# CX9898/BSMR-SDDMM

Hardware: AMD Instinct MI355X
Metric: SDDMM GFLOP/s (higher is better)
Workload: dtype f16

## Files before the change

### bsmr-sddmm_amd/csrc/gemm_kernels.hpp

```cpp
#pragma once

#include <hip/hip_runtime.h>
#include <stdint.h>

#include "gemm_format.hpp"
#include "sddmm_kernels.hpp"

namespace bsmr {

constexpr uint32_t kGemmBK = 64;
constexpr uint32_t kGemmRowBytes = kGemmBK * 2u;
__host__ __device__ constexpr uint32_t gemmSwz16(uint32_t row) { return (row >> 1) & 7u; }
__host__ __device__ constexpr uint32_t gemmSwz32(uint32_t row) { return ((row >> 1) & 1u) | (((row >> 3) & 1u) * 6u); }
constexpr uint32_t gemmStageBytes(int PM, int NB) { return (uint32_t)(PM + NB) * 16u * kGemmRowBytes; }
constexpr uint32_t kGemmSlabBytes = kGemmPassTiles * 1024u;
constexpr uint32_t gemmRingBytes(int PM, int NB) {
    return 2u * gemmStageBytes(PM, NB) > kGemmWaves * kGemmSlabBytes ? 2u * gemmStageBytes(PM, NB) : kGemmWaves * kGemmSlabBytes;
}
constexpr size_t gemmLdsBytes(int PM, int NB) { return gemmRingBytes(PM, NB) + (size_t)PM * 16u * 4u; }

#if defined(BSMR_GEMM_LAB)
#define GEMM_LAB_ARG , uint32_t labSkip, unsigned long long* labStamps
#define GEMM_LAB_SKIP(bit) (labSkip & (1u << (bit)))
#define GEMM_LAB_STAMPS unsigned long long labStamp[8] = {0, 0, 0, 0, 0, 0, 0, 0}
#define GEMM_LAB_STAMP(i) labStamp[i] = __builtin_amdgcn_s_memrealtime()
#define GEMM_LAB_STAMPS_OUT                                                                              \
    if (labStamps && lane == 0)                                                                          \
        for (uint32_t i = 0; i < 8u; ++i) labStamps[((size_t)blockIdx.x * kGemmWaves + wave) * 8u + i] = labStamp[i]
#else
#define GEMM_LAB_ARG
#define GEMM_LAB_SKIP(bit) false
#define GEMM_LAB_STAMPS
#define GEMM_LAB_STAMP(i)
#define GEMM_LAB_STAMPS_OUT
#endif

__device__ __forceinline__ void gemmKeep(const u32x4& x) {
#if defined(__HIP_DEVICE_COMPILE__)
    asm volatile("" ::"v"(x));
#else
    (void)x;
#endif
}

constexpr uint32_t kGemmDumpHigh = 64764u;
__device__ __forceinline__ void gemmDumpTile(const f32x4& a, uint32_t tileAddr, bool high) {
#if defined(__HIP_DEVICE_COMPILE__)
#pragma clang diagnostic push
#pragma clang diagnostic ignored "-Winline-asm"
    if (!high)
        asm volatile("s_mov_b32 m0, %4\n\ts_nop 0\n\tds_write_addtid_b32 %0\n\tds_write_addtid_b32 %1 offset:256\n\t"
                     "ds_write_addtid_b32 %2 offset:512\n\tds_write_addtid_b32 %3 offset:768"
                     ::"v"(a[0]), "v"(a[1]), "v"(a[2]), "v"(a[3]), "s"(tileAddr) : "memory", "m0");
    else
        asm volatile("s_mov_b32 m0, %4\n\ts_nop 0\n\tds_write_addtid_b32 %0 offset:64764\n\tds_write_addtid_b32 %1 offset:65020\n\t"
                     "ds_write_addtid_b32 %2 offset:65276\n\tds_write_addtid_b32 %3 offset:65532"
                     ::"v"(a[0]), "v"(a[1]), "v"(a[2]), "v"(a[3]), "s"(tileAddr - kGemmDumpHigh) : "memory", "m0");
#pragma clang diagnostic pop
#else
    (void)a; (void)tileAddr; (void)high;
#endif
}
__device__ __forceinline__ uint32_t gemmLdsAddress(const void* p) {
    return (uint32_t)(uintptr_t)(__attribute__((address_space(3))) const void*)p;
}

template <uint32_t DMAS>
__device__ __forceinline__ void gemmStagePart(const uint8_t* src, uint32_t srcBytes, uint8_t* dst, uint32_t wave, const uint32_t* voff, uint32_t kOff) {
    const auto rsrc = __builtin_amdgcn_make_buffer_rsrc(const_cast<uint8_t*>(src), 0, srcBytes, 0x00020000);
#pragma unroll
    for (uint32_t j = 0; j < DMAS; ++j)
        __builtin_amdgcn_raw_ptr_buffer_load_lds(rsrc, (__attribute__((address_space(3))) void*)(dst + (wave * DMAS + j) * 1024u), 16, voff[j], kOff, 0, 0);
}
__device__ __forceinline__ void gemmStoreEntry(float* P, bool live, uint32_t index, float val) {
    const auto rsrc = __builtin_amdgcn_make_buffer_rsrc(P, 0, 0xFFFFFFFC, 0x00020000);
    __builtin_amdgcn_raw_buffer_store_b32(__builtin_bit_cast(uint32_t, val), rsrc, live ? index << 2 : 0xFFFFFFFFu, 0, 0);
}
template <uint32_t C>
__device__ __forceinline__ void gemmLoadWords(const uint32_t* __restrict__ words, uint32_t e0, uint32_t lane, uint32_t (&w)[C], bool skip) {
    const uint32_t* __restrict__ base = words + e0;
#pragma unroll
    for (uint32_t u = 0; u < C; ++u) w[u] = skip ? kGemmNoEntry : base[u * kWave + lane];
}
template <uint32_t C, uint32_t HALF>
__device__ __forceinline__ void gemmMaskTrip(const float* slab, const uint32_t* rowTable, float* P, uint32_t e, uint32_t last, uint32_t lane,
                                             const uint32_t (&w)[C], bool skipStores) {
#pragma unroll
    for (uint32_t u = 0; u < C; ++u) {
        const bool live = e + u * kWave + lane < last && w[u] != kGemmNoEntry;
        const float val = slab[w[u] & 4095u];
        const uint32_t dst = rowTable[(w[u] >> 12) & (HALF - 1u)] + (w[u] >> 19);
        if (!skipStores) gemmStoreEntry(P, live, dst, val);
    }
}
template <uint32_t C, uint32_t HALF, uint32_t Q, bool DEEP>
__device__ __forceinline__ void gemmMaskPass(const uint32_t* __restrict__ words, const float* slab, const uint32_t* rowTable, float* P,
                                             const uint32_t (&myList)[Q + 1u], uint32_t q, uint32_t lane, uint32_t (&wAhead)[2][C],
                                             bool skipLoads, bool skipStores) {
    const uint32_t first = myList[q], last = myList[q + 1u];
    uint32_t w[C];
#pragma unroll
    for (uint32_t u = 0; u < C; ++u) w[u] = wAhead[q & 1u][u];
    if (DEEP) {
        if (q + 2u < Q) gemmLoadWords<C>(words, myList[q + 2u], lane, wAhead[q & 1u], skipLoads);
    } else if (q + 1u < Q) {
        gemmLoadWords<C>(words, last, lane, wAhead[(q + 1u) & 1u], skipLoads);
    }
    constexpr uint32_t T = C * kWave;
    const bool more = first + T < last;
    uint32_t over[C];
    if (more) gemmLoadWords<C>(words, first + T, lane, over, skipLoads);
    gemmMaskTrip<C, HALF>(slab, rowTable, P, first, last, lane, w, skipStores);
    if (more) {
        for (uint32_t e = first + T; e < last; e += T) {
            uint32_t ahead[C];
            gemmLoadWords<C>(words, e + T, lane, ahead, skipLoads);
            gemmMaskTrip<C, HALF>(slab, rowTable, P, e, last, lane, over, skipStores);
#pragma unroll
            for (uint32_t u = 0; u < C; ++u) over[u] = ahead[u];
        }
    }
}
template <uint32_t ADMAS, uint32_t BDMAS>
__device__ __forceinline__ void gemmStage(const uint8_t* A, uint32_t aBytes, const uint8_t* B, uint32_t bBytes, uint8_t* stage, uint32_t bAt,
                                          uint32_t wave, const uint32_t* voffA, const uint32_t* voffB, uint32_t kOff) {
    gemmStagePart<BDMAS>(B, bBytes, stage + bAt, wave, voffB, kOff);
    gemmStagePart<ADMAS>(A, aBytes, stage, wave, voffA, kOff);
}
__device__ __forceinline__ uint32_t gemmRowOfLane(const uint32_t* __restrict__ rows8, uint32_t sub) {
    uint32_t id = rows8[0];
#pragma unroll
    for (uint32_t k = 1; k < 8; ++k) id = sub == k ? rows8[k] : id;
    return id;
}

template <int KT, int PM, int NB, int MODE, bool SRC32 = false>
__global__ void __launch_bounds__(kGemmWaves * kWave, 2)
denseGemm(const void* __restrict__ Aop, const void* __restrict__ Bop, uint32_t aBytes, uint32_t bBytes,
          const uint32_t* __restrict__ panelRows, const uint32_t* __restrict__ colOf, const GemmItem* __restrict__ items,
          const uint32_t* __restrict__ rowStart,
          const uint32_t* __restrict__ lists, const uint32_t* __restrict__ words, float* __restrict__ P, uint32_t N,
          uint32_t gridG, uint32_t gridS, uint32_t fullGrid, Batch batch GEMM_LAB_ARG) {
    constexpr uint32_t ESZ = SRC32 ? 4u : 2u, K = (kGemmRowBytes / ESZ) * KT, TM = PM * 16u, TN = NB * 16u;
    constexpr uint32_t KSUB = SRC32 ? 1u : 2u;
    constexpr uint32_t m = PM / kGemmWavesM, n = NB / kGemmWavesN, Q = (m * n + kGemmPassTiles - 1u) / kGemmPassTiles, L = kGemmWaves * Q;
    constexpr uint32_t ADMAS = PM / 4u, BDMAS = NB / 4u;
    static_assert(PM % 4 == 0 && NB % 4 == 0, "a stage is filled in whole 1-KiB pieces per wave");
    constexpr uint32_t stageBytes = gemmStageBytes(PM, NB), bAt = TM * kGemmRowBytes;
    constexpr uint32_t rowTableAt = gemmRingBytes(PM, NB);
    constexpr uint32_t kGemmWordChunk = m * n > 32u ? 4u : 8u;
    constexpr bool kPlainDump = m * n > 32u;

    extern __shared__ __attribute__((aligned(16))) uint8_t lds[];
    const uint32_t itemId = xcdContiguous(blockIdx.x, gridDim.x);
    uint32_t group, firstBlock, listBase;
    if (fullGrid) {
        gemmItemPlace(itemId, gridG, gridS, group, firstBlock);
        firstBlock *= (uint32_t)NB;
        listBase = itemId * (L + 1u);
    } else {
        const GemmItem item = items[itemId];
        group = item.group;
        firstBlock = item.firstBlock;
        listBase = item.listBase;
    }
    const uint32_t wave = __builtin_amdgcn_readfirstlane(threadIdx.x >> 6), lane = threadIdx.x & 63u;
    const uint32_t wm = wave / kGemmWavesN, wn = wave % kGemmWavesN;
    const uint32_t r = lane & 15u, g = lane >> 4;
    GEMM_LAB_STAMPS;
    GEMM_LAB_STAMP(0);

    const uint8_t* Ab = static_cast<const uint8_t*>(Aop) + (size_t)blockIdx.y * batch.strideA * ESZ;
    const uint8_t* Bb = static_cast<const uint8_t*>(Bop) + (size_t)blockIdx.y * batch.strideB * ESZ;
    P += (size_t)blockIdx.y * batch.strideP;

    uint32_t voffA[ADMAS], voffB[BDMAS];
#pragma unroll
    for (uint32_t j = 0; j < BDMAS; ++j) {
        const uint32_t col = 8u * (wave * BDMAS + j) + (lane >> 3);
        const uint32_t id = gemmRowOfLane(colOf + (size_t)firstBlock * 16u + 8u * (wave * BDMAS + j), lane >> 3);
        voffB[j] = id * (K * ESZ) + (((lane & 7u) ^ (SRC32 ? gemmSwz32(col) : gemmSwz16(col))) << 4);
    }
    if (!GEMM_LAB_SKIP(2)) gemmStagePart<BDMAS>(Bb, bBytes, lds + bAt, wave, voffB, 0u);
#pragma unroll
    for (uint32_t j = 0; j < ADMAS; ++j) {
        const uint32_t row = 8u * (wave * ADMAS + j) + (lane >> 3);
        const uint32_t id = gemmRowOfLane(panelRows + (size_t)group * TM + 8u * (wave * ADMAS + j), lane >> 3);
        voffA[j] = id * (K * ESZ) + (((lane & 7u) ^ (SRC32 ? gemmSwz32(row) : gemmSwz16(row))) << 4);
    }
    if (!GEMM_LAB_SKIP(2)) gemmStagePart<ADMAS>(Ab, aBytes, lds, wave, voffA, 0u);
    GEMM_LAB_STAMP(1);
    if (threadIdx.x < TM) reinterpret_cast<uint32_t*>(lds + rowTableAt)[threadIdx.x] = rowStart[(size_t)itemId * TM + threadIdx.x];
    uint32_t myList[Q + 1];
#pragma unroll
    for (uint32_t q = 0; q <= Q; ++q) myList[q] = lists[listBase + wave * Q + q];

    const uint32_t fragOff = r * kGemmRowBytes + ((SRC32 ? (2u * g) ^ gemmSwz32(r) : g ^ gemmSwz16(r)) << 4);
    const uint32_t aRead = wm * (TM / 2u) * kGemmRowBytes + fragOff;
    const uint32_t bRead = bAt + wn * (TN / 4u) * kGemmRowBytes + fragOff;

    f32x4 acc[m][n];
#pragma unroll
    for (uint32_t i = 0; i < m; ++i)
#pragma unroll
        for (uint32_t j = 0; j < n; ++j) acc[i][j] = f32x4{0.f, 0.f, 0.f, 0.f};

    auto loadWords = [&](uint32_t e0, uint32_t (&w)[kGemmWordChunk]) { gemmLoadWords<kGemmWordChunk>(words, e0, lane, w, GEMM_LAB_SKIP(4)); };
    constexpr bool kDeepWords = Q >= 2u && m * n <= 32u;
    uint32_t wAhead[2][kGemmWordChunk];
    constexpr bool kEarlyWords = KT <= 4 && !kPlainDump;
    auto firstWords = [&]() {
        loadWords(myList[0], wAhead[0]);
        if (kDeepWords) loadWords(myList[1], wAhead[1]);
    };
#if !defined(BSMR_GEMM_LATE_WORDS)
    if (kEarlyWords) firstWords();
#endif

    asm volatile("s_waitcnt vmcnt(0)" ::: "memory");
    GEMM_LAB_STAMP(2);
    __builtin_amdgcn_s_barrier();
    GEMM_LAB_STAMP(3);
#if defined(BSMR_GEMM_LATE_WORDS)
    if (kEarlyWords) firstWords();
#endif

#pragma unroll
    for (uint32_t t = 0; t < (uint32_t)KT; ++t) {
        if (t + 1u < (uint32_t)KT && !GEMM_LAB_SKIP(2))
            gemmStage<ADMAS, BDMAS>(Ab, aBytes, Bb, bBytes, lds + ((t + 1u) & 1u) * stageBytes, bAt, wave, voffA, voffB, (t + 1u) * kGemmRowBytes);
        if (!kEarlyWords && t + 1u == (uint32_t)KT) firstWords();
        const uint8_t* base = lds + (t & 1u) * stageBytes;
#pragma unroll
        for (uint32_t s = 0; s < KSUB; ++s) {
            auto fragment = [&](uint32_t at, uint32_t tile, uint32_t tag) -> u32x4 {
                if (GEMM_LAB_SKIP(1)) return u32x4{lane, t, tile, s + tag};
                const uint8_t* src = base + ((at + tile * 16u * kGemmRowBytes) ^ (s << 6));
                if constexpr (SRC32) {
                    const f32x4 lo = *reinterpret_cast<const f32x4*>(src);
                    const f32x4 hi = *reinterpret_cast<const f32x4*>(reinterpret_cast<const uint8_t*>(reinterpret_cast<uintptr_t>(src) ^ 16u));
                    return packLowp<MODE>(lo, hi);
                } else {
                    return *reinterpret_cast<const u32x4*>(src);
                }
            };
            u32x4 bf[n];
#pragma unroll
            for (uint32_t j = 0; j < n; ++j) bf[j] = fragment(bRead, j, 0u);
#pragma unroll
            for (uint32_t i = 0; i < m; ++i) {
                const u32x4 af = fragment(aRead, i, 2u);
                if (!GEMM_LAB_SKIP(0)) {
#pragma unroll
                    for (uint32_t j = 0; j < n; ++j) acc[i][j] = mfma16<MODE>(af, bf[j], acc[i][j]);
                } else {
                    gemmKeep(af);
#pragma unroll
                    for (uint32_t j = 0; j < n; ++j) gemmKeep(bf[j]);
                }
            }
        }
        asm volatile("s_waitcnt vmcnt(0) lgkmcnt(0)" ::: "memory");
        __builtin_amdgcn_s_barrier();
    }

    GEMM_LAB_STAMP(4);
    float* slab = reinterpret_cast<float*>(lds) + wave * (kGemmPassTiles * 256u);
    const uint32_t slabAddr = __builtin_amdgcn_readfirstlane(gemmLdsAddress(slab));
    const uint32_t* rowTable = reinterpret_cast<const uint32_t*>(lds + rowTableAt) + wm * (TM / 2u);
#pragma unroll
    for (uint32_t q = 0; q < Q; ++q) {
        if (!GEMM_LAB_SKIP(3)) {
            if (kPlainDump) {
#pragma unroll
                for (uint32_t tp = 0; tp < kGemmPassTiles; ++tp) {
                    const uint32_t tIdx = q * kGemmPassTiles + tp;
                    if (tIdx < m * n) {
#pragma unroll
                        for (uint32_t j = 0; j < 4u; ++j) slab[tp * 256u + j * 64u + lane] = acc[tIdx / n][tIdx % n][j];
                    }
                }
            } else if (slabAddr < 0x10000u) {
#pragma unroll
                for (uint32_t tp = 0; tp < kGemmPassTiles; ++tp) {
                    const uint32_t tIdx = q * kGemmPassTiles + tp;
                    if (tIdx < m * n) gemmDumpTile(acc[tIdx / n][tIdx % n], slabAddr + tp * 1024u, false);
                }
            } else {
#pragma unroll
                for (uint32_t tp = 0; tp < kGemmPassTiles; ++tp) {
                    const uint32_t tIdx = q * kGemmPassTiles + tp;
                    if (tIdx < m * n) gemmDumpTile(acc[tIdx / n][tIdx % n], slabAddr + tp * 1024u, true);
                }
            }
        }
        if (kPlainDump) __builtin_amdgcn_sched_barrier(0);
        gemmMaskPass<kGemmWordChunk, TM / 2u, Q, kDeepWords>(words, slab, rowTable, P, myList, q, lane, wAhead, GEMM_LAB_SKIP(4), GEMM_LAB_SKIP(5));
        GEMM_LAB_STAMP(5u + q);
    }
    GEMM_LAB_STAMPS_OUT;
}

constexpr uint32_t kGemmHalfRowBytes = 64u;
__host__ __device__ constexpr uint32_t gemmSwzH(uint32_t row) { return (4u - ((row >> 2) & 3u)) & 3u; }
constexpr uint32_t gemmCvtRingBytes(int PM, int NB) {
    const uint32_t used = (uint32_t)(PM + NB) * 16u * (kGemmRowBytes + 2u * kGemmHalfRowBytes);
    return used > kGemmWaves * kGemmSlabBytes ? used : kGemmWaves * kGemmSlabBytes;
}
constexpr size_t gemmCvtLdsBytes(int PM, int NB) { return gemmCvtRingBytes(PM, NB) + (size_t)PM * 16u * 4u; }

template <int KT, int PM, int NB, int MODE>
__global__ void __launch_bounds__(kGemmWaves * kWave, 2)
denseGemmCvt(const float* __restrict__ Aop, const float* __restrict__ Bop, uint32_t aBytes, uint32_t bBytes,
             const uint32_t* __restrict__ panelRows, const uint32_t* __restrict__ colOf, const GemmItem* __restrict__ items,
             const uint32_t* __restrict__ rowStart,
             const uint32_t* __restrict__ lists, const uint32_t* __restrict__ words, float* __restrict__ P, uint32_t N,
             uint32_t gridG, uint32_t gridS, uint32_t fullGrid, Batch batch GEMM_LAB_ARG) {
    constexpr uint32_t K = 32u * KT, TM = PM * 16u, TN = NB * 16u, ROWS = TM + TN;
    constexpr uint32_t m = PM / kGemmWavesM, n = NB / kGemmWavesN, Q = (m * n + kGemmPassTiles - 1u) / kGemmPassTiles, L = kGemmWaves * Q;
    constexpr uint32_t ADMAS = PM / 4u, BDMAS = NB / 4u, DMAS = ADMAS + BDMAS;
    constexpr uint32_t fBytes = ROWS * kGemmRowBytes, hBytes = ROWS * kGemmHalfRowBytes, bAtF = TM * kGemmRowBytes, bAtH = TM * kGemmHalfRowBytes;
    constexpr uint32_t hAt = fBytes, rowTableAt = gemmCvtRingBytes(PM, NB);
    constexpr uint32_t kGemmWordChunk = m * n > 32u ? 4u : 8u;

    extern __shared__ __attribute__((aligned(16))) uint8_t lds[];
    const uint32_t itemId = xcdContiguous(blockIdx.x, gridDim.x);
    uint32_t group, firstBlock, listBase;
    if (fullGrid) {
        gemmItemPlace(itemId, gridG, gridS, group, firstBlock);
        firstBlock *= (uint32_t)NB;
        listBase = itemId * (L + 1u);
    } else {
        const GemmItem item = items[itemId];
        group = item.group;
        firstBlock = item.firstBlock;
        listBase = item.listBase;
    }
    const uint32_t wave = __builtin_amdgcn_readfirstlane(threadIdx.x >> 6), lane = threadIdx.x & 63u;
    const uint32_t wm = wave / kGemmWavesN, wn = wave % kGemmWavesN;
    const uint32_t r = lane & 15u, g = lane >> 4;
    GEMM_LAB_STAMPS;
    GEMM_LAB_STAMP(0);
    const uint8_t* Ab = reinterpret_cast<const uint8_t*>(Aop) + (size_t)blockIdx.y * batch.strideA * 4u;
    const uint8_t* Bb = reinterpret_cast<const uint8_t*>(Bop) + (size_t)blockIdx.y * batch.strideB * 4u;
    P += (size_t)blockIdx.y * batch.strideP;

    uint32_t voffA[ADMAS], voffB[BDMAS];
    const uint32_t piece = lane & 7u;
#pragma unroll
    for (uint32_t j = 0; j < BDMAS; ++j)
        voffB[j] = gemmRowOfLane(colOf + (size_t)firstBlock * 16u + 8u * (wave * BDMAS + j), lane >> 3) * (K * 4u) + (piece << 4);
    if (!GEMM_LAB_SKIP(2)) gemmStagePart<BDMAS>(Bb, bBytes, lds + bAtF, wave, voffB, 0u);
#pragma unroll
    for (uint32_t j = 0; j < ADMAS; ++j)
        voffA[j] = gemmRowOfLane(panelRows + (size_t)group * TM + 8u * (wave * ADMAS + j), lane >> 3) * (K * 4u) + (piece << 4);
    if (!GEMM_LAB_SKIP(2)) gemmStagePart<ADMAS>(Ab, aBytes, lds, wave, voffA, 0u);
    GEMM_LAB_STAMP(1);
    if (threadIdx.x < TM) reinterpret_cast<uint32_t*>(lds + rowTableAt)[threadIdx.x] = rowStart[(size_t)itemId * TM + threadIdx.x];
    uint32_t myList[Q + 1];
#pragma unroll
    for (uint32_t q = 0; q <= Q; ++q) myList[q] = lists[listBase + wave * Q + q];

#if defined(BSMR_GEMM_ROUND_SERIAL)
    constexpr uint32_t kRoundBatch = 1u;
#else
    constexpr uint32_t kRoundBatch = 5u;
#endif
    const uint32_t fOfA = wave * ADMAS * 1024u + lane * 16u, fOfB = bAtF + wave * BDMAS * 1024u + lane * 16u;
    auto hOf = [&](uint32_t part, uint32_t firstChunk, uint32_t odd) {
        const uint32_t quarter = (2u * (firstChunk + odd) + (lane >> 5)) & 3u;
        return hAt + part + firstChunk * 512u + (lane >> 3) * kGemmHalfRowBytes + (((piece >> 1) ^ ((4u - quarter) & 3u)) << 4) + ((piece & 1u) << 3);
    };
    const uint32_t hOfA[2] = {hOf(0u, wave * ADMAS, 0u), hOf(0u, wave * ADMAS, 1u)};
    const uint32_t hOfB[2] = {hOf(bAtH, wave * BDMAS, 0u), hOf(bAtH, wave * BDMAS, 1u)};
    auto roundChunks = [&](uint32_t to) {
        if (GEMM_LAB_SKIP(1)) return;
#pragma unroll
        for (uint32_t j0 = 0; j0 < DMAS; j0 += kRoundBatch) {
            f32x4 v[kRoundBatch];
#pragma unroll
            for (uint32_t b = 0; b < kRoundBatch; ++b) {
                const uint32_t j = j0 + b;
                if (j >= DMAS) continue;
                v[b] = j < ADMAS ? *reinterpret_cast<const f32x4*>(lds + fOfA + j * 1024u)
                                 : *reinterpret_cast<const f32x4*>(lds + fOfB + (j - ADMAS) * 1024u);
            }
#pragma unroll
            for (uint32_t b = 0; b < kRoundBatch; ++b) {
                const uint32_t j = j0 + b;
                if (j >= DMAS) continue;
                const uint32_t jj = j < ADMAS ? j : j - ADMAS;
                uint8_t* dst = lds + (j < ADMAS ? hOfA[jj & 1u] : hOfB[jj & 1u]) + jj * 512u + to * hBytes;
                typedef uint32_t u32x2 __attribute__((ext_vector_type(2)));
                u32x2 h;
                if constexpr (MODE == 0) {
                    typedef _Float16 f16x4 __attribute__((ext_vector_type(4)));
                    f16x4 o;
                    o[0] = (_Float16)v[b][0]; o[1] = (_Float16)v[b][1]; o[2] = (_Float16)v[b][2]; o[3] = (_Float16)v[b][3];
                    h = __builtin_bit_cast(u32x2, o);
                } else {
                    typedef __bf16 bf16x4 __attribute__((ext_vector_type(4)));
                    bf16x4 o;
                    o[0] = (__bf16)v[b][0]; o[1] = (__bf16)v[b][1]; o[2] = (__bf16)v[b][2]; o[3] = (__bf16)v[b][3];
                    h = __builtin_bit_cast(u32x2, o);
                }
                *reinterpret_cast<u32x2*>(dst) = h;
            }
        }
    };

    const uint32_t fragOff = r * kGemmHalfRowBytes + ((g ^ gemmSwzH(r)) << 4);
    const uint32_t aRead = wm * (TM / 2u) * kGemmHalfRowBytes + fragOff;
    const uint32_t bRead = bAtH + wn * (TN / 4u) * kGemmHalfRowBytes + fragOff;

    f32x4 acc[m][n];
#pragma unroll
    for (uint32_t i = 0; i < m; ++i)
#pragma unroll
        for (uint32_t j = 0; j < n; ++j) acc[i][j] = f32x4{0.f, 0.f, 0.f, 0.f};
    auto loadWords = [&](uint32_t e0, uint32_t (&w)[kGemmWordChunk]) { gemmLoadWords<kGemmWordChunk>(words, e0, lane, w, GEMM_LAB_SKIP(4)); };
    constexpr bool kDeepWords = Q >= 2u && m * n <= 32u;
    uint32_t wAhead[2][kGemmWordChunk];
    constexpr bool kEarlyWords = KT <= 4;
    auto firstWords = [&]() {
        loadWords(myList[0], wAhead[0]);
        if (kDeepWords) loadWords(myList[1], wAhead[1]);
    };
#if !defined(BSMR_GEMM_LATE_WORDS)
    if (kEarlyWords) firstWords();
#endif

    asm volatile("s_waitcnt vmcnt(0)" ::: "memory");
    GEMM_LAB_STAMP(2);
    roundChunks(0u);
    asm volatile("s_waitcnt lgkmcnt(0)" ::: "memory");
    if (KT > 1 && !GEMM_LAB_SKIP(2)) gemmStage<ADMAS, BDMAS>(Ab, aBytes, Bb, bBytes, lds, bAtF, wave, voffA, voffB, kGemmRowBytes);
    __builtin_amdgcn_s_barrier();
    GEMM_LAB_STAMP(3);
#if defined(BSMR_GEMM_LATE_WORDS)
    if (kEarlyWords) firstWords();
#endif

#pragma unroll
    for (uint32_t t = 0; t < (uint32_t)KT; ++t) {
        if (!kEarlyWords && t + 1u == (uint32_t)KT) firstWords();
        const uint8_t* base = lds + hAt + (t & 1u) * hBytes;
        u32x4 bf[n];
#pragma unroll
        for (uint32_t j = 0; j < n; ++j)
            bf[j] = GEMM_LAB_SKIP(6) ? u32x4{lane, t, j, 0u} : *reinterpret_cast<const u32x4*>(base + bRead + j * 16u * kGemmHalfRowBytes);
#pragma unroll
        for (uint32_t i = 0; i < m; ++i) {
            const u32x4 af = GEMM_LAB_SKIP(6) ? u32x4{lane, t, i, 2u} : *reinterpret_cast<const u32x4*>(base + aRead + i * 16u * kGemmHalfRowBytes);
            if (!GEMM_LAB_SKIP(0)) {
#pragma unroll
                for (uint32_t j = 0; j < n; ++j) acc[i][j] = mfma16<MODE>(af, bf[j], acc[i][j]);
            } else {
                gemmKeep(af);
#pragma unroll
                for (uint32_t j = 0; j < n; ++j) gemmKeep(bf[j]);
            }
        }
        if (t + 1u < (uint32_t)KT) {
            asm volatile("s_waitcnt vmcnt(0)" ::: "memory");
            roundChunks((t + 1u) & 1u);
            asm volatile("s_waitcnt lgkmcnt(0)" ::: "memory");
            if (t + 2u < (uint32_t)KT && !GEMM_LAB_SKIP(2))
                gemmStage<ADMAS, BDMAS>(Ab, aBytes, Bb, bBytes, lds, bAtF, wave, voffA, voffB, (t + 2u) * kGemmRowBytes);
        } else {
            asm volatile("s_waitcnt lgkmcnt(0)" ::: "memory");
        }
        __builtin_amdgcn_s_barrier();
    }

    GEMM_LAB_STAMP(4);
    float* slab = reinterpret_cast<float*>(lds) + wave * (kGemmPassTiles * 256u);
    const uint32_t slabAddr = __builtin_amdgcn_readfirstlane(gemmLdsAddress(slab));
    const uint32_t* rowTable = reinterpret_cast<const uint32_t*>(lds + rowTableAt) + wm * (TM / 2u);
#pragma unroll
    for (uint32_t q = 0; q < Q; ++q) {
        if (!GEMM_LAB_SKIP(3)) {
            if (slabAddr < 0x10000u) {
#pragma unroll
                for (uint32_t tp = 0; tp < kGemmPassTiles; ++tp) {
                    const uint32_t tIdx = q * kGemmPassTiles + tp;
                    if (tIdx < m * n) gemmDumpTile(acc[tIdx / n][tIdx % n], slabAddr + tp * 1024u, false);
                }
            } else {
#pragma unroll
                for (uint32_t tp = 0; tp < kGemmPassTiles; ++tp) {
                    const uint32_t tIdx = q * kGemmPassTiles + tp;
                    if (tIdx < m * n) gemmDumpTile(acc[tIdx / n][tIdx % n], slabAddr + tp * 1024u, true);
                }
            }
        }
        gemmMaskPass<kGemmWordChunk, TM / 2u, Q, kDeepWords>(words, slab, rowTable, P, myList, q, lane, wAhead, GEMM_LAB_SKIP(4), GEMM_LAB_SKIP(5));
        GEMM_LAB_STAMP(5u + q);
    }
    GEMM_LAB_STAMPS_OUT;
}

}
```

Baseline: 15620.

## Load A fp32 slices straight into registers and deepen B staging pipeline

The fp32-input GEMM kernel no longer stages A through LDS. A slices are loaded with buffer loads directly into registers and converted to half when they land, while B keeps an fp32 double buffer in LDS and is now prefetched two slices ahead. Waits use partial vmcnt counts instead of draining everything, and the rowStart table write is deferred. This targets the full vmcnt(0) stalls and the extra LDS round trip for A, at the cost of more VGPRs, a different LDS footprint, and new lab timing spans.

```diff
diff --git a/bsmr-sddmm_amd/csrc/gemm_kernels.hpp b/bsmr-sddmm_amd/csrc/gemm_kernels.hpp
--- a/bsmr-sddmm_amd/csrc/gemm_kernels.hpp
+++ b/bsmr-sddmm_amd/csrc/gemm_kernels.hpp
@@ -20,18 +20,23 @@
 constexpr size_t gemmLdsBytes(int PM, int NB) { return gemmRingBytes(PM, NB) + (size_t)PM * 16u * 4u; }
 
 #if defined(BSMR_GEMM_LAB)
+constexpr uint32_t kGemmLabStamps = 10;
 #define GEMM_LAB_ARG , uint32_t labSkip, unsigned long long* labStamps
 #define GEMM_LAB_SKIP(bit) (labSkip & (1u << (bit)))
-#define GEMM_LAB_STAMPS unsigned long long labStamp[8] = {0, 0, 0, 0, 0, 0, 0, 0}
+#define GEMM_LAB_STAMPS unsigned long long labStamp[kGemmLabStamps] = {0, 0, 0, 0, 0, 0, 0, 0, 0, 0}, labSpan = 0
 #define GEMM_LAB_STAMP(i) labStamp[i] = __builtin_amdgcn_s_memrealtime()
+#define GEMM_LAB_SPAN_BEGIN labSpan = __builtin_amdgcn_s_memrealtime()
+#define GEMM_LAB_SPAN_END(i) labStamp[i] += __builtin_amdgcn_s_memrealtime() - labSpan
 #define GEMM_LAB_STAMPS_OUT                                                                              \
     if (labStamps && lane == 0)                                                                          \
-        for (uint32_t i = 0; i < 8u; ++i) labStamps[((size_t)blockIdx.x * kGemmWaves + wave) * 8u + i] = labStamp[i]
+        for (uint32_t i = 0; i < kGemmLabStamps; ++i) labStamps[((size_t)blockIdx.x * kGemmWaves + wave) * kGemmLabStamps + i] = labStamp[i]
 #else
 #define GEMM_LAB_ARG
 #define GEMM_LAB_SKIP(bit) false
 #define GEMM_LAB_STAMPS
 #define GEMM_LAB_STAMP(i)
+#define GEMM_LAB_SPAN_BEGIN
+#define GEMM_LAB_SPAN_END(i)
 #define GEMM_LAB_STAMPS_OUT
 #endif
 
@@ -304,10 +309,45 @@
 constexpr uint32_t kGemmHalfRowBytes = 64u;
 __host__ __device__ constexpr uint32_t gemmSwzH(uint32_t row) { return (4u - ((row >> 2) & 3u)) & 3u; }
 constexpr uint32_t gemmCvtRingBytes(int PM, int NB) {
-    const uint32_t used = (uint32_t)(PM + NB) * 16u * (kGemmRowBytes + 2u * kGemmHalfRowBytes);
+    const uint32_t used = 2u * (uint32_t)NB * 16u * kGemmRowBytes + 2u * (uint32_t)(PM + NB) * 16u * kGemmHalfRowBytes;
     return used > kGemmWaves * kGemmSlabBytes ? used : kGemmWaves * kGemmSlabBytes;
 }
 constexpr size_t gemmCvtLdsBytes(int PM, int NB) { return gemmCvtRingBytes(PM, NB) + (size_t)PM * 16u * 4u; }
+static_assert(gemmCvtLdsBytes(16, 20) <= 160u * 1024u && gemmCvtLdsBytes(16, 16) <= 160u * 1024u && gemmCvtLdsBytes(8, 20) <= 160u * 1024u &&
+              gemmCvtLdsBytes(8, 16) <= 160u * 1024u, "the fp32 kernel's LDS fits a CU's 160 KiB");
+
+template <uint32_t CHUNKS>
+__device__ __forceinline__ void gemmLoadChunks(const uint8_t* src, uint32_t srcBytes, const uint32_t* voff, uint32_t kOff, f32x4 (&v)[CHUNKS]) {
+    const auto rsrc = __builtin_amdgcn_make_buffer_rsrc(const_cast<uint8_t*>(src), 0, srcBytes, 0x00020000);
+#pragma unroll
+    for (uint32_t j = 0; j < CHUNKS; ++j) v[j] = __builtin_bit_cast(f32x4, __builtin_amdgcn_raw_buffer_load_b128(rsrc, voff[j], kOff, 0));
+}
+template <uint32_t N, uint32_t CHUNKS>
+__device__ __forceinline__ void gemmWaitRequests(f32x4 (&landed)[CHUNKS]) {
+    static_assert(N < 64u, "vmcnt holds six bits");
+    asm volatile("s_waitcnt vmcnt(%0)" ::"n"(N) : "memory");
+#if defined(__HIP_DEVICE_COMPILE__)
+#pragma unroll
+    for (uint32_t j = 0; j < CHUNKS; ++j) asm volatile("" : "+v"(landed[j]));
+#endif
+}
+template <int MODE>
+__device__ __forceinline__ void gemmRoundPiece(const f32x4& v, uint8_t* dst) {
+    typedef uint32_t u32x2 __attribute__((ext_vector_type(2)));
+    u32x2 h;
+    if constexpr (MODE == 0) {
+        typedef _Float16 f16x4 __attribute__((ext_vector_type(4)));
+        f16x4 o;
+        o[0] = (_Float16)v[0]; o[1] = (_Float16)v[1]; o[2] = (_Float16)v[2]; o[3] = (_Float16)v[3];
+        h = __builtin_bit_cast(u32x2, o);
+    } else {
+        typedef __bf16 bf16x4 __attribute__((ext_vector_type(4)));
+        bf16x4 o;
+        o[0] = (__bf16)v[0]; o[1] = (__bf16)v[1]; o[2] = (__bf16)v[2]; o[3] = (__bf16)v[3];
+        h = __builtin_bit_cast(u32x2, o);
+    }
+    *reinterpret_cast<u32x2*>(dst) = h;
+}
 
 template <int KT, int PM, int NB, int MODE>
 __global__ void __launch_bounds__(kGemmWaves * kWave, 2)
@@ -318,9 +358,10 @@
              uint32_t gridG, uint32_t gridS, uint32_t fullGrid, Batch batch GEMM_LAB_ARG) {
     constexpr uint32_t K = 32u * KT, TM = PM * 16u, TN = NB * 16u, ROWS = TM + TN;
     constexpr uint32_t m = PM / kGemmWavesM, n = NB / kGemmWavesN, Q = (m * n + kGemmPassTiles - 1u) / kGemmPassTiles, L = kGemmWaves * Q;
-    constexpr uint32_t ADMAS = PM / 4u, BDMAS = NB / 4u, DMAS = ADMAS + BDMAS;
-    constexpr uint32_t fBytes = ROWS * kGemmRowBytes, hBytes = ROWS * kGemmHalfRowBytes, bAtF = TM * kGemmRowBytes, bAtH = TM * kGemmHalfRowBytes;
-    constexpr uint32_t hAt = fBytes, rowTableAt = gemmCvtRingBytes(PM, NB);
+    constexpr uint32_t ADMAS = PM / 4u, BDMAS = NB / 4u;
+    constexpr uint32_t fBytes = TN * kGemmRowBytes, hBytes = ROWS * kGemmHalfRowBytes, bAtH = TM * kGemmHalfRowBytes;
+    constexpr uint32_t hAt = 2u * fBytes, rowTableAt = gemmCvtRingBytes(PM, NB);
+    static_assert(hAt + 2u * hBytes <= rowTableAt, "F's two stages and H's two lie in front of the row table");
     constexpr uint32_t kGemmWordChunk = m * n > 32u ? 4u : 8u;
 
     extern __shared__ __attribute__((aligned(16))) uint8_t lds[];
@@ -348,65 +389,50 @@
     uint32_t voffA[ADMAS], voffB[BDMAS];
     const uint32_t piece = lane & 7u;
 #pragma unroll
+    for (uint32_t j = 0; j < ADMAS; ++j)
+        voffA[j] = gemmRowOfLane(panelRows + (size_t)group * TM + 8u * (wave * ADMAS + j), lane >> 3) * (K * 4u) + (piece << 4);
+#pragma unroll
     for (uint32_t j = 0; j < BDMAS; ++j)
         voffB[j] = gemmRowOfLane(colOf + (size_t)firstBlock * 16u + 8u * (wave * BDMAS + j), lane >> 3) * (K * 4u) + (piece << 4);
-    if (!GEMM_LAB_SKIP(2)) gemmStagePart<BDMAS>(Bb, bBytes, lds + bAtF, wave, voffB, 0u);
-#pragma unroll
-    for (uint32_t j = 0; j < ADMAS; ++j)
-        voffA[j] = gemmRowOfLane(panelRows + (size_t)group * TM + 8u * (wave * ADMAS + j), lane >> 3) * (K * 4u) + (piece << 4);
-    if (!GEMM_LAB_SKIP(2)) gemmStagePart<ADMAS>(Ab, aBytes, lds, wave, voffA, 0u);
+    uint32_t myRowStart = 0;
+    if (threadIdx.x < TM) myRowStart = rowStart[(size_t)itemId * TM + threadIdx.x];
+    f32x4 aNext[ADMAS];
+#pragma unroll
+    for (uint32_t j = 0; j < ADMAS; ++j) aNext[j] = f32x4{0.f, 0.f, 0.f, 0.f};
+    auto requestA = [&](uint32_t slice) {
+        __builtin_amdgcn_sched_barrier(0);
+        if (slice < (uint32_t)KT && !GEMM_LAB_SKIP(2)) gemmLoadChunks<ADMAS>(Ab, aBytes, voffA, slice * kGemmRowBytes, aNext);
+        __builtin_amdgcn_sched_barrier(0);
+    };
+    auto requestB = [&](uint32_t slice) {
+        __builtin_amdgcn_sched_barrier(0);
+        if (slice < (uint32_t)KT && !GEMM_LAB_SKIP(2)) gemmStagePart<BDMAS>(Bb, bBytes, lds + (slice & 1u) * fBytes, wave, voffB, slice * kGemmRowBytes);
+        __builtin_amdgcn_sched_barrier(0);
+    };
+    requestA(0u);
+    requestB(0u);
     GEMM_LAB_STAMP(1);
-    if (threadIdx.x < TM) reinterpret_cast<uint32_t*>(lds + rowTableAt)[threadIdx.x] = rowStart[(size_t)itemId * TM + threadIdx.x];
     uint32_t myList[Q + 1];
 #pragma unroll
     for (uint32_t q = 0; q <= Q; ++q) myList[q] = lists[listBase + wave * Q + q];
 
-#if defined(BSMR_GEMM_ROUND_SERIAL)
-    constexpr uint32_t kRoundBatch = 1u;
-#else
-    constexpr uint32_t kRoundBatch = 5u;
-#endif
-    const uint32_t fOfA = wave * ADMAS * 1024u + lane * 16u, fOfB = bAtF + wave * BDMAS * 1024u + lane * 16u;
+    const uint32_t fOfB = wave * BDMAS * 1024u + lane * 16u;
     auto hOf = [&](uint32_t part, uint32_t firstChunk, uint32_t odd) {
         const uint32_t quarter = (2u * (firstChunk + odd) + (lane >> 5)) & 3u;
         return hAt + part + firstChunk * 512u + (lane >> 3) * kGemmHalfRowBytes + (((piece >> 1) ^ ((4u - quarter) & 3u)) << 4) + ((piece & 1u) << 3);
     };
     const uint32_t hOfA[2] = {hOf(0u, wave * ADMAS, 0u), hOf(0u, wave * ADMAS, 1u)};
     const uint32_t hOfB[2] = {hOf(bAtH, wave * BDMAS, 0u), hOf(bAtH, wave * BDMAS, 1u)};
-    auto roundChunks = [&](uint32_t to) {
+    auto roundChunks = [&](uint32_t slice) {
         if (GEMM_LAB_SKIP(1)) return;
-#pragma unroll
-        for (uint32_t j0 = 0; j0 < DMAS; j0 += kRoundBatch) {
-            f32x4 v[kRoundBatch];
-#pragma unroll
-            for (uint32_t b = 0; b < kRoundBatch; ++b) {
-                const uint32_t j = j0 + b;
-                if (j >= DMAS) continue;
-                v[b] = j < ADMAS ? *reinterpret_cast<const f32x4*>(lds + fOfA + j * 1024u)
-                                 : *reinterpret_cast<const f32x4*>(lds + fOfB + (j - ADMAS) * 1024u);
-            }
-#pragma unroll
-            for (uint32_t b = 0; b < kRoundBatch; ++b) {
-                const uint32_t j = j0 + b;
-                if (j >= DMAS) continue;
-                const uint32_t jj = j < ADMAS ? j : j - ADMAS;
-                uint8_t* dst = lds + (j < ADMAS ? hOfA[jj & 1u] : hOfB[jj & 1u]) + jj * 512u + to * hBytes;
-                typedef uint32_t u32x2 __attribute__((ext_vector_type(2)));
-                u32x2 h;
-                if constexpr (MODE == 0) {
-                    typedef _Float16 f16x4 __attribute__((ext_vector_type(4)));
-                    f16x4 o;
-                    o[0] = (_Float16)v[b][0]; o[1] = (_Float16)v[b][1]; o[2] = (_Float16)v[b][2]; o[3] = (_Float16)v[b][3];
-                    h = __builtin_bit_cast(u32x2, o);
-                } else {
-                    typedef __bf16 bf16x4 __attribute__((ext_vector_type(4)));
-                    bf16x4 o;
-                    o[0] = (__bf16)v[b][0]; o[1] = (__bf16)v[b][1]; o[2] = (__bf16)v[b][2]; o[3] = (__bf16)v[b][3];
-                    h = __builtin_bit_cast(u32x2, o);
-                }
-                *reinterpret_cast<u32x2*>(dst) = h;
-            }
-        }
+        const uint32_t to = (slice & 1u) * hBytes;
+        f32x4 v[BDMAS];
+#pragma unroll
+        for (uint32_t j = 0; j < BDMAS; ++j) v[j] = *reinterpret_cast<const f32x4*>(lds + (slice & 1u) * fBytes + fOfB + j * 1024u);
+#pragma unroll
+        for (uint32_t j = 0; j < ADMAS; ++j) gemmRoundPiece<MODE>(aNext[j], lds + hOfA[j & 1u] + j * 512u + to);
+#pragma unroll
+        for (uint32_t j = 0; j < BDMAS; ++j) gemmRoundPiece<MODE>(v[j], lds + hOfB[j & 1u] + j * 512u + to);
     };
 
     const uint32_t fragOff = r * kGemmHalfRowBytes + ((g ^ gemmSwzH(r)) << 4);
@@ -421,7 +447,7 @@
     auto loadWords = [&](uint32_t e0, uint32_t (&w)[kGemmWordChunk]) { gemmLoadWords<kGemmWordChunk>(words, e0, lane, w, GEMM_LAB_SKIP(4)); };
     constexpr bool kDeepWords = Q >= 2u && m * n <= 32u;
     uint32_t wAhead[2][kGemmWordChunk];
-    constexpr bool kEarlyWords = KT <= 4;
+    constexpr bool kEarlyWords = KT <= 4 && m * n <= 32u;
     auto firstWords = [&]() {
         loadWords(myList[0], wAhead[0]);
         if (kDeepWords) loadWords(myList[1], wAhead[1]);
@@ -430,11 +456,14 @@
     if (kEarlyWords) firstWords();
 #endif
 
-    asm volatile("s_waitcnt vmcnt(0)" ::: "memory");
+    requestB(1u);
+    if (KT > 1) gemmWaitRequests<BDMAS>(aNext); else gemmWaitRequests<0>(aNext);
     GEMM_LAB_STAMP(2);
+    if (threadIdx.x < TM) reinterpret_cast<uint32_t*>(lds + rowTableAt)[threadIdx.x] = myRowStart;
     roundChunks(0u);
     asm volatile("s_waitcnt lgkmcnt(0)" ::: "memory");
-    if (KT > 1 && !GEMM_LAB_SKIP(2)) gemmStage<ADMAS, BDMAS>(Ab, aBytes, Bb, bBytes, lds, bAtF, wave, voffA, voffB, kGemmRowBytes);
+    requestA(1u);
+    requestB(2u);
     __builtin_amdgcn_s_barrier();
     GEMM_LAB_STAMP(3);
 #if defined(BSMR_GEMM_LATE_WORDS)
@@ -443,7 +472,10 @@
 
 #pragma unroll
     for (uint32_t t = 0; t < (uint32_t)KT; ++t) {
-        if (!kEarlyWords && t + 1u == (uint32_t)KT) firstWords();
+        if (!kEarlyWords && t + 1u == (uint32_t)KT) {
+            firstWords();
+            __builtin_amdgcn_sched_barrier(0);
+        }
         const uint8_t* base = lds + hAt + (t & 1u) * hBytes;
         u32x4 bf[n];
 #pragma unroll
@@ -451,6 +483,13 @@
             bf[j] = GEMM_LAB_SKIP(6) ? u32x4{lane, t, j, 0u} : *reinterpret_cast<const u32x4*>(base + bRead + j * 16u * kGemmHalfRowBytes);
 #pragma unroll
         for (uint32_t i = 0; i < m; ++i) {
+            if (i + 1u == m && t + 1u < (uint32_t)KT) {
+                __builtin_amdgcn_sched_barrier(0);
+                GEMM_LAB_SPAN_BEGIN;
+                if (t + 2u < (uint32_t)KT) gemmWaitRequests<BDMAS>(aNext); else gemmWaitRequests<0>(aNext);
+                GEMM_LAB_SPAN_END(8);
+                GEMM_LAB_SPAN_BEGIN;
+            }
             const u32x4 af = GEMM_LAB_SKIP(6) ? u32x4{lane, t, i, 2u} : *reinterpret_cast<const u32x4*>(base + aRead + i * 16u * kGemmHalfRowBytes);
             if (!GEMM_LAB_SKIP(0)) {
 #pragma unroll
@@ -462,15 +501,16 @@
             }
         }
         if (t + 1u < (uint32_t)KT) {
-            asm volatile("s_waitcnt vmcnt(0)" ::: "memory");
-            roundChunks((t + 1u) & 1u);
+            roundChunks(t + 1u);
             asm volatile("s_waitcnt lgkmcnt(0)" ::: "memory");
-            if (t + 2u < (uint32_t)KT && !GEMM_LAB_SKIP(2))
-                gemmStage<ADMAS, BDMAS>(Ab, aBytes, Bb, bBytes, lds, bAtF, wave, voffA, voffB, (t + 2u) * kGemmRowBytes);
+            requestA(t + 2u);
+            requestB(t + 3u);
         } else {
             asm volatile("s_waitcnt lgkmcnt(0)" ::: "memory");
+            GEMM_LAB_SPAN_BEGIN;
         }
         __builtin_amdgcn_s_barrier();
+        GEMM_LAB_SPAN_END(9);
     }
 
     GEMM_LAB_STAMP(4);
```

Result: faster. 16840 (median of 6 runs) (+7.8%).
